# jhqxxx/aha

Hardware: AMD Instinct MI355X
Metric: decode tokens/s (greedy, batch 1) -- Qwen3-VL-8B, 1x1024^2 image + 512-token prompt; prefill tok/s alongside (higher is better)
Workload: dtype bf16; 1 GPU; qwen3vl8b; image=1024, kv_len_mid=2024, replicas=1, loop=device-resident greedy loop

## Files before the change

aha_amd/csrc/kernels_vit.hip:

```cpp
#include "common.h"
#include "kernels.h"

namespace aha {

template <int VPL>
__global__ __launch_bounds__(256) void layernorm_rows_kernel(const bf16_t* __restrict__ x, const bf16_t* __restrict__ w,
                                                             const bf16_t* __restrict__ b, bf16_t* __restrict__ y,
                                                             int64_t rows, int dim, float eps) {
  const int lane = threadIdx.x & 63;
  const int64_t row = (int64_t)blockIdx.x * 4 + (threadIdx.x >> 6);
  if (row >= rows) return;
  const bf16_t* xr = x + row * dim;
  bf16_t* yr = y + row * dim;
  const int nvec = dim / 8;
  float f[VPL][8];
  float s = 0.f;
#pragma unroll
  for (int i = 0; i < VPL; ++i) {
    const int vi = i * 64 + lane;
    if (vi < nvec) {
      const u32x4_t v = ld16(xr + vi * 8);
#pragma unroll
      for (int j = 0; j < 4; ++j) { f[i][2 * j] = lo_bf(v[j]); f[i][2 * j + 1] = hi_bf(v[j]); }
#pragma unroll
      for (int j = 0; j < 8; ++j) s += f[i][j];
    }
  }
  const float mean = wave_sum(s) / (float)dim;
  float q = 0.f;
#pragma unroll
  for (int i = 0; i < VPL; ++i) {
    const int vi = i * 64 + lane;
    if (vi < nvec) {
#pragma unroll
      for (int j = 0; j < 8; ++j) { const float d = f[i][j] - mean; q += d * d; }
    }
  }
  const float rstd = 1.0f / sqrtf(wave_sum(q) / (float)dim + eps);
#pragma unroll
  for (int i = 0; i < VPL; ++i) {
    const int vi = i * 64 + lane;
    if (vi < nvec) {
      const u32x4_t wv = ld16(w + vi * 8), bv = ld16(b + vi * 8);
      u32x4_t o;
#pragma unroll
      for (int j = 0; j < 4; ++j)
        o[j] = pack_bf((f[i][2 * j] - mean) * rstd * lo_bf(wv[j]) + lo_bf(bv[j]),
                       (f[i][2 * j + 1] - mean) * rstd * hi_bf(wv[j]) + hi_bf(bv[j]));
      *reinterpret_cast<u32x4_t*>(yr + vi * 8) = o;
    }
  }
}
void launch_layernorm_rows(const void* x, const void* w, const void* b, void* y, int64_t rows, int dim, float eps,
                           hipStream_t st) {
  if (rows <= 0) return;
  dim3 grid((unsigned)((rows + 3) / 4)), block(256);
  const int vpl = (dim / 8 + 63) / 64;
#define LN_CASE(V)                                                                                                   \
  hipLaunchKernelGGL(layernorm_rows_kernel<V>, grid, block, 0, st, (const bf16_t*)x, (const bf16_t*)w, (const bf16_t*)b, \
                     (bf16_t*)y, rows, dim, eps)
  if (vpl <= 1) LN_CASE(1);
  else if (vpl <= 3) LN_CASE(3);
  else if (vpl <= 9) LN_CASE(9);
  else LN_CASE(16);
#undef LN_CASE
}

__global__ __launch_bounds__(256) void pos_embed_add_kernel(bf16_t* __restrict__ x, const bf16_t* __restrict__ table,
                                                            const int32_t* __restrict__ idx, const float* __restrict__ wt,
                                                            int64_t N, int D) {
  const int64_t n = blockIdx.x;
  const bf16_t* e[4];
  float w[4];
#pragma unroll
  for (int i = 0; i < 4; ++i) {
    e[i] = table + (int64_t)idx[i * N + n] * D;
    w[i] = rbf(wt[i * N + n]);
  }
  bf16_t* xr = x + n * D;
  for (int v = threadIdx.x; v < D / 8; v += 256) {
    u32x4_t ev[4];
#pragma unroll
    for (int i = 0; i < 4; ++i) ev[i] = ld16(e[i] + v * 8);
    const u32x4_t xv = ld16(xr + v * 8);
    u32x4_t o;
#pragma unroll
    for (int j = 0; j < 4; ++j) {
      float lo = rbf(lo_bf(ev[0][j]) * w[0]), hi = rbf(hi_bf(ev[0][j]) * w[0]);
#pragma unroll
      for (int i = 1; i < 4; ++i) {
        lo = rbf(lo + rbf(lo_bf(ev[i][j]) * w[i]));
        hi = rbf(hi + rbf(hi_bf(ev[i][j]) * w[i]));
      }
      o[j] = pack_bf(lo_bf(xv[j]) + lo, hi_bf(xv[j]) + hi);
    }
    *reinterpret_cast<u32x4_t*>(xr + v * 8) = o;
  }
}
void launch_pos_embed_add(void* x, const void* table, const int32_t* idx, const float* wt, int64_t N, int D,
                          hipStream_t st) {
  if (N <= 0) return;
  hipLaunchKernelGGL(pos_embed_add_kernel, dim3((unsigned)N), dim3(256), 0, st, (bf16_t*)x, (const bf16_t*)table, idx, wt, N, D);
}

__global__ __launch_bounds__(256) void vit_rope_pack_kernel(VitRopeArgs a, int n_qk_blocks) {
  const int lane = threadIdx.x & 63;
  const int hd = a.hd, half = hd / 2;
  const int D = a.nh * hd;
  if ((int)blockIdx.x < n_qk_blocks) {
    const int64_t wid = (int64_t)blockIdx.x * 4 + (threadIdx.x >> 6);
    const int64_t unit = wid * 7 + lane / 9;
    const int g = lane % 9;
    if (lane >= 63 || unit >= (int64_t)a.N * 2) return;
    const int which = (int)(unit & 1), n = (int)(unit >> 1);
    const int e0 = 4 * g;
    const float4 cs01 = *reinterpret_cast<const float4*>(a.cs_tab + ((int64_t)n * half + e0) * 2);
    const float4 cs23 = *reinterpret_cast<const float4*>(a.cs_tab + ((int64_t)n * half + e0 + 2) * 2);
    const float c[4] = {cs01.x, cs01.z, cs23.x, cs23.z}, s[4] = {cs01.y, cs01.w, cs23.y, cs23.w};
    const bf16_t* src = (const bf16_t*)a.qkv + (int64_t)n * 3 * D + (int64_t)which * D + e0;
    bf16_t* dq = (bf16_t*)a.q_out + (int64_t)n * a.nh * VIT_DQK;
    const int slot = a.slot_of[n];
    bf16_t* dk = reinterpret_cast<bf16_t*>(a.kv.page_ptrs[a.page_of[n]] + a.kv.layer_off);
    const int k0 = kpage_elem(slot, e0, VIT_DQK / 32), k1 = kpage_elem(slot, e0 + half, VIT_DQK / 32), kz = kpage_elem(slot, hd + 4 * (g % 6), VIT_DQK / 32);
    const uint2 zero = {0u, 0u};
    for (int h0 = 0; h0 < a.nh; h0 += 4) {
      uint2 x0w[4], x1w[4];
#pragma unroll
      for (int i = 0; i < 4; ++i)
        if (h0 + i < a.nh) {
          x0w[i] = *reinterpret_cast<const uint2*>(src + (int64_t)(h0 + i) * hd);
          x1w[i] = *reinterpret_cast<const uint2*>(src + (int64_t)(h0 + i) * hd + half);
        }
#pragma unroll
      for (int i = 0; i < 4; ++i) {
        const int h = h0 + i;
        if (h >= a.nh) break;
        const float x0[4] = {lo_bf(x0w[i].x), hi_bf(x0w[i].x), lo_bf(x0w[i].y), hi_bf(x0w[i].y)};
        const float x1[4] = {lo_bf(x1w[i].x), hi_bf(x1w[i].x), lo_bf(x1w[i].y), hi_bf(x1w[i].y)};
        float y0[4], y1[4];
#pragma unroll
        for (int j = 0; j < 4; ++j) {
          y0[j] = rbf(x0[j] * c[j]) + rbf(-x1[j] * s[j]);
          y1[j] = rbf(x1[j] * c[j]) + rbf(x0[j] * s[j]);
        }
        const uint2 o0 = {pack_bf(y0[0], y0[1]), pack_bf(y0[2], y0[3])}, o1 = {pack_bf(y1[0], y1[1]), pack_bf(y1[2], y1[3])};
        if (which == 0) {
          bf16_t* qd = dq + (int64_t)h * VIT_DQK;
          *reinterpret_cast<uint2*>(qd + e0) = o0;
          *reinterpret_cast<uint2*>(qd + e0 + half) = o1;
          if (g < (VIT_DQK - 72) / 4) *reinterpret_cast<uint2*>(qd + hd + 4 * g) = zero;
        } else {
          bf16_t* kd = dk + (int64_t)h * KV_PAGE_TOKENS * VIT_DQK;
          *reinterpret_cast<uint2*>(kd + k0) = o0;
          *reinterpret_cast<uint2*>(kd + k1) = o1;
          if (g < (VIT_DQK - 72) / 4) *reinterpret_cast<uint2*>(kd + kz) = zero;
        }
      }
    }
    return;
  }
  const int64_t u = (int64_t)(blockIdx.x - n_qk_blocks) * 256 + threadIdx.x;
  const int64_t unit = u / 80;
  const int lu = (int)(u % 80);
  if (unit >= (int64_t)a.n_pages * a.nh) return;
  const int page = (int)(unit / a.nh), h = (int)(unit % a.nh);
  const int kk = lu / 40, G = (lu % 40) / 10, dchunk = lu % 10;
  const int first = a.page_first[page], cnt = a.page_cnt[page];
  uint32_t in[8][4];
#pragma unroll
  for (int e = 0; e < 8; ++e) {
    const int tslot = kk * 32 + (e >> 2) * 16 + G * 4 + (e & 3);
    u32x4_t v = {0u, 0u, 0u, 0u};
    if (tslot < cnt && dchunk < 9)
      v = ld16((const bf16_t*)a.qkv + (int64_t)(first + tslot) * 3 * D + 2 * (int64_t)D + (int64_t)h * hd + dchunk * 8);
    if (tslot < cnt && dchunk == 9) v[0] = 0x3F80u;
    in[e][0] = v[0]; in[e][1] = v[1]; in[e][2] = v[2]; in[e][3] = v[3];
  }
  bf16_t* vd = reinterpret_cast<bf16_t*>(a.kv.page_ptrs[page] + a.kv.layer_off) + (int64_t)a.nh * KV_PAGE_TOKENS * VIT_DQK +
               (int64_t)h * VIT_DV * KV_PAGE_TOKENS;
#pragma unroll
  for (int dd = 0; dd < 8; ++dd) {
    const int d = dchunk * 8 + dd;
    u32x4_t o;
#pragma unroll
    for (int w = 0; w < 4; ++w) {
      const uint32_t a0 = in[2 * w][dd >> 1], a1 = in[2 * w + 1][dd >> 1];
      o[w] = (dd & 1) ? ((a0 >> 16) | (a1 & 0xffff0000u)) : ((a0 & 0xffffu) | (a1 << 16));
    }
    *reinterpret_cast<u32x4_t*>(vd + ((((d >> 4) * 2 + kk) * 64 + G * 16 + (d & 15)) << 3)) = o;
  }
}
__global__ __launch_bounds__(256) void vit_rope_table_kernel(const int32_t* __restrict__ rowcol, const float* __restrict__ inv_freq, int N,
                                                             int hd, float* __restrict__ tab) {
  const int half = hd / 2, quarter = hd / 4;
  const int64_t g = (int64_t)blockIdx.x * 256 + threadIdx.x;
  if (g >= (int64_t)N * half) return;
  const int n = (int)(g / half), lane = (int)(g % half);
  const int pos = (lane < quarter) ? rowcol[2 * n] : rowcol[2 * n + 1];
  const float ang = (float)pos * inv_freq[lane % quarter];
  tab[g * 2] = rbf(cosf(ang));
  tab[g * 2 + 1] = rbf(sinf(ang));
}
void launch_vit_rope_table(const int32_t* rowcol, const float* inv_freq, int N, int hd, float* tab, hipStream_t st) {
  if (N <= 0) return;
  hipLaunchKernelGGL(vit_rope_table_kernel, dim3((unsigned)(((int64_t)N * (hd / 2) + 255) / 256)), dim3(256), 0, st, rowcol, inv_freq, N, hd, tab);
}
void launch_vit_rope_pack(const VitRopeArgs& a, hipStream_t st) {
  if (a.N <= 0) return;
  const int64_t units = (int64_t)a.N * 2, waves = (units + 6) / 7;
  const int n_qk_blocks = (int)((waves + 3) / 4);
  const int n_v_blocks = (int)(((int64_t)a.n_pages * a.nh * 80 + 255) / 256);
  hipLaunchKernelGGL(vit_rope_pack_kernel, dim3((unsigned)(n_qk_blocks + n_v_blocks)), dim3(256), 0, st, a, n_qk_blocks);
}

__global__ __launch_bounds__(256) void scatter_rows_kernel(bf16_t* __restrict__ dst, const bf16_t* __restrict__ src,
                                                           const int32_t* __restrict__ rows, int D, int add) {
  const int64_t i = blockIdx.x;
  bf16_t* d = dst + (int64_t)rows[i] * D;
  const bf16_t* s = src + i * D;
  for (int v = threadIdx.x; v < D / 8; v += 256) {
    u32x4_t sv = ld16(s + v * 8);
    if (add) {
      const u32x4_t dv = ld16(d + v * 8);
#pragma unroll
      for (int j = 0; j < 4; ++j) sv[j] = pack_bf(lo_bf(dv[j]) + lo_bf(sv[j]), hi_bf(dv[j]) + hi_bf(sv[j]));
    }
    *reinterpret_cast<u32x4_t*>(d + v * 8) = sv;
  }
}
void launch_scatter_rows(void* dst, const void* src, const int32_t* rows, int64_t n, int D, int add, hipStream_t st) {
  if (n <= 0) return;
  hipLaunchKernelGGL(scatter_rows_kernel, dim3((unsigned)n), dim3(256), 0, st, (bf16_t*)dst, (const bf16_t*)src, rows, D, add);
}

}

namespace aha {
__global__ __launch_bounds__(192) void image_to_patches_kernel(const uint8_t* __restrict__ img, bf16_t* __restrict__ out,
                                                               int H, int W, int patch, int merge, float m0, float m1,
                                                               float m2, float s0, float s1, float s2) {
  const int gw = W / patch, bwn = gw / merge;
  const int n = blockIdx.x;
  const int iw = n % merge, ih = (n / merge) % merge, bw = (n / (merge * merge)) % bwn, bh = n / (merge * merge * bwn);
  const int y0 = (bh * merge + ih) * patch, x0 = (bw * merge + iw) * patch;
  const int pp = patch * patch;
  const float inv255 = 1.0f / 255.0f;
  for (int e = threadIdx.x; e < 3 * pp; e += blockDim.x) {
    const int c = e / pp, py = (e % pp) / patch, px = e % patch;
    const float mean = c == 0 ? m0 : (c == 1 ? m1 : m2), sd = c == 0 ? s0 : (c == 1 ? s1 : s2);
    const float v = (float)img[((size_t)(y0 + py) * W + (x0 + px)) * 3 + c];
    const bf16_t b = f2bf((v * inv255 + 0.0f - mean) / sd);
    bf16_t* o = out + (size_t)n * (6 * pp) + (size_t)c * 2 * pp + py * patch + px;
    o[0] = b;
    o[pp] = b;
  }
}
__global__ __launch_bounds__(192) void video_to_patches_kernel(const uint8_t* __restrict__ frames, bf16_t* __restrict__ out, int T,
                                                               int H, int W, int patch, int merge, float m0, float m1, float m2,
                                                               float s0, float s1, float s2) {
  const int gw = W / patch, gh = H / patch, bwn = gw / merge;
  const int t = blockIdx.x / (gh * gw), n = blockIdx.x % (gh * gw);
  const int iw = n % merge, ih = (n / merge) % merge, bw = (n / (merge * merge)) % bwn, bh = n / (merge * merge * bwn);
  const int y0 = (bh * merge + ih) * patch, x0 = (bw * merge + iw) * patch;
  const int pp = patch * patch;
  const float inv255 = rbf(1.0f / 255.0f);
  for (int e = threadIdx.x; e < 3 * pp; e += blockDim.x) {
    const int c = e / pp, py = (e % pp) / patch, px = e % patch;
    const float mean = rbf(c == 0 ? m0 : (c == 1 ? m1 : m2)), sd = rbf(c == 0 ? s0 : (c == 1 ? s1 : s2));
    bf16_t* o = out + (size_t)blockIdx.x * (6 * pp) + (size_t)c * 2 * pp + py * patch + px;
#pragma unroll
    for (int k = 0; k < 2; ++k) {
      const int f = min(2 * t + k, T - 1);
      const float v = (float)frames[(((size_t)f * H + (y0 + py)) * W + (x0 + px)) * 3 + c];
      o[k * pp] = f2bf(rbf(rbf(rbf(v * inv255) + 0.0f) - mean) / sd);
    }
  }
}
void launch_video_to_patches(const uint8_t* frames, void* out, int T, int H, int W, int patch, int merge, const float* mean,
                             const float* stdv, hipStream_t st) {
  const int n = ((T + 1) / 2) * (H / patch) * (W / patch);
  if (n <= 0) return;
  hipLaunchKernelGGL(video_to_patches_kernel, dim3(n), dim3(192), 0, st, frames, (bf16_t*)out, T, H, W, patch, merge, mean[0],
                     mean[1], mean[2], stdv[0], stdv[1], stdv[2]);
}
void launch_image_to_patches(const uint8_t* img, void* out, int H, int W, int patch, int merge, const float* mean,
                             const float* stdv, hipStream_t st) {
  const int n = (H / patch) * (W / patch);
  if (n <= 0) return;
  hipLaunchKernelGGL(image_to_patches_kernel, dim3(n), dim3(192), 0, st, img, (bf16_t*)out, H, W, patch, merge, mean[0],
                     mean[1], mean[2], stdv[0], stdv[1], stdv[2]);
}
}
```

Baseline: 346.7 tokens/s.

## Restructure ViT rope-pack: 16-byte vectors, head-group split, global-address-space stores

Reworks the ViT RoPE pack kernel so each lane handles 8 contiguous elements with 16-byte loads and stores instead of two 8-byte halves. The rotate-half partner is fetched separately and its sign is flipped with an XOR. Work is also split across head groups of 8 per wavefront, giving more waves and less serial per-wave looping. Stores go through an explicit global address-space pointer to get global store instructions. This only affects vision-encoder prefill, so decode tokens/s should barely move; it adds more partner loads per element and more complex indexing.

```diff
diff --git a/aha_amd/csrc/kernels_vit.hip b/aha_amd/csrc/kernels_vit.hip
--- a/aha_amd/csrc/kernels_vit.hip
+++ b/aha_amd/csrc/kernels_vit.hip
@@ -103,58 +103,67 @@
   hipLaunchKernelGGL(pos_embed_add_kernel, dim3((unsigned)N), dim3(256), 0, st, (bf16_t*)x, (const bf16_t*)table, idx, wt, N, D);
 }
 
+constexpr int VIT_ROPE_HEADS_PER_UNIT = 8;
+typedef __attribute__((address_space(1))) u32x4_t* gst16_t;
 __global__ __launch_bounds__(256) void vit_rope_pack_kernel(VitRopeArgs a, int n_qk_blocks) {
   const int lane = threadIdx.x & 63;
   const int hd = a.hd, half = hd / 2;
   const int D = a.nh * hd;
   if ((int)blockIdx.x < n_qk_blocks) {
-    const int64_t wid = (int64_t)blockIdx.x * 4 + (threadIdx.x >> 6);
-    const int64_t unit = wid * 7 + lane / 9;
-    const int g = lane % 9;
-    if (lane >= 63 || unit >= (int64_t)a.N * 2) return;
-    const int which = (int)(unit & 1), n = (int)(unit >> 1);
-    const int e0 = 4 * g;
-    const float4 cs01 = *reinterpret_cast<const float4*>(a.cs_tab + ((int64_t)n * half + e0) * 2);
-    const float4 cs23 = *reinterpret_cast<const float4*>(a.cs_tab + ((int64_t)n * half + e0 + 2) * 2);
-    const float c[4] = {cs01.x, cs01.z, cs23.x, cs23.z}, s[4] = {cs01.y, cs01.w, cs23.y, cs23.w};
-    const bf16_t* src = (const bf16_t*)a.qkv + (int64_t)n * 3 * D + (int64_t)which * D + e0;
-    bf16_t* dq = (bf16_t*)a.q_out + (int64_t)n * a.nh * VIT_DQK;
-    const int slot = a.slot_of[n];
-    bf16_t* dk = reinterpret_cast<bf16_t*>(a.kv.page_ptrs[a.page_of[n]] + a.kv.layer_off);
-    const int k0 = kpage_elem(slot, e0, VIT_DQK / 32), k1 = kpage_elem(slot, e0 + half, VIT_DQK / 32), kz = kpage_elem(slot, hd + 4 * (g % 6), VIT_DQK / 32);
-    const uint2 zero = {0u, 0u};
-    for (int h0 = 0; h0 < a.nh; h0 += 4) {
-      uint2 x0w[4], x1w[4];
+    constexpr int hpu = VIT_ROPE_HEADS_PER_UNIT;
+    const int n_hg = (a.nh + hpu - 1) / hpu;
+    const int64_t wid = (int64_t)blockIdx.x * 4 + (threadIdx.x >> 6), tg = wid / n_hg;
+    const int hbeg = (int)(wid % n_hg) * hpu, hend = min(hbeg + hpu, a.nh);
+    const int which = (int)(tg & 1);
+    const int64_t n = (tg >> 1) * 7 + lane / 9;
+    const int j = lane % 9;
+    if (lane >= 63 || n >= a.N) return;
+    const bool firstA = 8 * j < half, firstB = 8 * j + 4 < half;
+    const int mA = firstA ? 8 * j : 8 * j - half, mB = firstB ? 8 * j + 4 : 8 * j + 4 - half;
+    const int pA = firstA ? mA + half : mA, pB = firstB ? mB + half : mB;
+    const float* tab = a.cs_tab + n * half * 2;
+    const float4 t0 = *reinterpret_cast<const float4*>(tab + mA * 2), t1 = *reinterpret_cast<const float4*>(tab + mA * 2 + 4);
+    const float4 t2 = *reinterpret_cast<const float4*>(tab + mB * 2), t3 = *reinterpret_cast<const float4*>(tab + mB * 2 + 4);
+    const float c[8] = {t0.x, t0.z, t1.x, t1.z, t2.x, t2.z, t3.x, t3.z}, s[8] = {t0.y, t0.w, t1.y, t1.w, t2.y, t2.w, t3.y, t3.w};
+    const uint32_t sgnA = firstA ? 0x80008000u : 0u, sgnB = firstB ? 0x80008000u : 0u;
+    const bf16_t* src = (const bf16_t*)a.qkv + n * 3 * D + (int64_t)which * D;
+    uint64_t dst, dpad;
+    int64_t hstride;
+    if (which == 0) {
+      dst = (uint64_t)a.q_out + (n * a.nh * VIT_DQK + 8 * j) * 2;
+      dpad = (uint64_t)a.q_out + (n * a.nh * VIT_DQK + hd + 8 * (j % 3)) * 2;
+      hstride = VIT_DQK * 2;
+    } else {
+      const int slot = a.slot_of[n];
+      const uint64_t page = a.kv.page_ptrs[a.page_of[n]] + a.kv.layer_off;
+      dst = page + (uint64_t)kpage_elem(slot, 8 * j, VIT_DQK / 32) * 2;
+      dpad = page + (uint64_t)kpage_elem(slot, hd + 8 * (j % 3), VIT_DQK / 32) * 2;
+      hstride = (int64_t)KV_PAGE_TOKENS * VIT_DQK * 2;
+    }
+    const u32x4_t zero = {0u, 0u, 0u, 0u};
+    for (int h0 = hbeg; h0 < hend; h0 += 4) {
+      u32x4_t xw[4];
+      uint2 paw[4], pbw[4];
 #pragma unroll
       for (int i = 0; i < 4; ++i)
-        if (h0 + i < a.nh) {
-          x0w[i] = *reinterpret_cast<const uint2*>(src + (int64_t)(h0 + i) * hd);
-          x1w[i] = *reinterpret_cast<const uint2*>(src + (int64_t)(h0 + i) * hd + half);
+        if (h0 + i < hend) {
+          const bf16_t* sh = src + (int64_t)(h0 + i) * hd;
+          xw[i] = ld16(sh + 8 * j);
+          paw[i] = *reinterpret_cast<const uint2*>(sh + pA);
+          pbw[i] = *reinterpret_cast<const uint2*>(sh + pB);
         }
 #pragma unroll
       for (int i = 0; i < 4; ++i) {
         const int h = h0 + i;
-        if (h >= a.nh) break;
-        const float x0[4] = {lo_bf(x0w[i].x), hi_bf(x0w[i].x), lo_bf(x0w[i].y), hi_bf(x0w[i].y)};
-        const float x1[4] = {lo_bf(x1w[i].x), hi_bf(x1w[i].x), lo_bf(x1w[i].y), hi_bf(x1w[i].y)};
-        float y0[4], y1[4];
-#pragma unroll
-        for (int j = 0; j < 4; ++j) {
-          y0[j] = rbf(x0[j] * c[j]) + rbf(-x1[j] * s[j]);
-          y1[j] = rbf(x1[j] * c[j]) + rbf(x0[j] * s[j]);
-        }
-        const uint2 o0 = {pack_bf(y0[0], y0[1]), pack_bf(y0[2], y0[3])}, o1 = {pack_bf(y1[0], y1[1]), pack_bf(y1[2], y1[3])};
-        if (which == 0) {
-          bf16_t* qd = dq + (int64_t)h * VIT_DQK;
-          *reinterpret_cast<uint2*>(qd + e0) = o0;
-          *reinterpret_cast<uint2*>(qd + e0 + half) = o1;
-          if (g < (VIT_DQK - 72) / 4) *reinterpret_cast<uint2*>(qd + hd + 4 * g) = zero;
-        } else {
-          bf16_t* kd = dk + (int64_t)h * KV_PAGE_TOKENS * VIT_DQK;
-          *reinterpret_cast<uint2*>(kd + k0) = o0;
-          *reinterpret_cast<uint2*>(kd + k1) = o1;
-          if (g < (VIT_DQK - 72) / 4) *reinterpret_cast<uint2*>(kd + kz) = zero;
-        }
+        if (h >= hend) break;
+        const uint32_t pw[4] = {paw[i].x ^ sgnA, paw[i].y ^ sgnA, pbw[i].x ^ sgnB, pbw[i].y ^ sgnB};
+        u32x4_t o;
+#pragma unroll
+        for (int w = 0; w < 4; ++w)
+          o[w] = pack_bf(rbf(lo_bf(xw[i][w]) * c[2 * w]) + rbf(lo_bf(pw[w]) * s[2 * w]),
+                         rbf(hi_bf(xw[i][w]) * c[2 * w + 1]) + rbf(hi_bf(pw[w]) * s[2 * w + 1]));
+        *reinterpret_cast<gst16_t>(dst + h * hstride) = o;
+        if (j < (VIT_DQK - 72) / 8) *reinterpret_cast<gst16_t>(dpad + h * hstride) = zero;
       }
     }
     return;
@@ -187,7 +196,7 @@
       const uint32_t a0 = in[2 * w][dd >> 1], a1 = in[2 * w + 1][dd >> 1];
       o[w] = (dd & 1) ? ((a0 >> 16) | (a1 & 0xffff0000u)) : ((a0 & 0xffffu) | (a1 << 16));
     }
-    *reinterpret_cast<u32x4_t*>(vd + ((((d >> 4) * 2 + kk) * 64 + G * 16 + (d & 15)) << 3)) = o;
+    *reinterpret_cast<gst16_t>((uint64_t)(vd + ((((d >> 4) * 2 + kk) * 64 + G * 16 + (d & 15)) << 3))) = o;
   }
 }
 __global__ __launch_bounds__(256) void vit_rope_table_kernel(const int32_t* __restrict__ rowcol, const float* __restrict__ inv_freq, int N,
@@ -207,7 +216,8 @@
 }
 void launch_vit_rope_pack(const VitRopeArgs& a, hipStream_t st) {
   if (a.N <= 0) return;
-  const int64_t units = (int64_t)a.N * 2, waves = (units + 6) / 7;
+  constexpr int hpu = VIT_ROPE_HEADS_PER_UNIT;
+  const int64_t waves = ((int64_t)a.N + 6) / 7 * 2 * ((a.nh + hpu - 1) / hpu);
   const int n_qk_blocks = (int)((waves + 3) / 4);
   const int n_v_blocks = (int)(((int64_t)a.n_pages * a.nh * 80 + 255) / 256);
   hipLaunchKernelGGL(vit_rope_pack_kernel, dim3((unsigned)(n_qk_blocks + n_v_blocks)), dim3(256), 0, st, a, n_qk_blocks);
```

Result: no change. 346.5 tokens/s (-0.1%).
